# kowaalczyk/reformer-tts

Measured on AMD Instinct MI355X. Metric: mel-frames/sec training step, LJSpeech-shape batch, higher is better.
Workload: dtype bf16; 1 GPU; config/baseline.yml full Reformer-TTS training step (enc 3 / dec 3 layers, d=512, LSH 8 rounds, buckets 64/128), per-GPU batch 12, text 200->256, mel 1024x80; global_batch=12, parallelism=dp1, reversible_recompute=full

## Files before the change

reformer-tts_amd/csrc/gemm_tn.hip:

```cpp
#include "rtts_common.h"
#include <stdlib.h>

#define GT_BM 64
#ifndef GT_PAD
#define GT_PAD 64
#endif

typedef __attribute__((ext_vector_type(8))) short gt_short8;

__device__ __forceinline__ bf16x8 gt_tr_frag(const unsigned char* p0, const unsigned char* p1) {
    const short4v lo = __builtin_amdgcn_ds_read_tr16_b64_v4i16((RTTS_LDS short4v*)p0);
    const short4v hi = __builtin_amdgcn_ds_read_tr16_b64_v4i16((RTTS_LDS short4v*)p1);
    const gt_short8 both = {lo[0], lo[1], lo[2], lo[3], hi[0], hi[1], hi[2], hi[3]};
    return __builtin_bit_cast(bf16x8, both);
}

struct GtProb {
    const bf16_t* a;
    const bf16_t* b;
    float* out;
    float* c;
    int64_t lda, ldb, ldo, ldc;
    size_t slab_stride;
    int M, N, K, split, accumulate;
    int wg_start;
    int rb_start;
};
struct GtGroup {
    GtProb p[RTTS_GEMM_TN_MAX_GROUP];
    int n;
};

template <int WN, int WK, int TN, int TK>
__global__ __launch_bounds__(64 * WN * WK) void gemm_tn_kernel(const GtGroup grp) {
    constexpr int BN = 32 * TN * WN, BK = 32 * TK * WK, NTHR = 64 * WN * WK;
    constexpr int ROWA = BN * 2 + GT_PAD, ROWB = BK * 2 + GT_PAD;
    constexpr int PA = BN / 8, PB = BK / 8;
    constexpr int ITA = GT_BM * PA / NTHR, ITB = GT_BM * PB / NTHR;
    static_assert(GT_BM * PA % NTHR == 0 && GT_BM * PB % NTHR == 0, "staging must tile");
    extern __shared__ __attribute__((aligned(16))) unsigned char smem[];
    unsigned char* As = smem;
    unsigned char* Bs = smem + 2 * GT_BM * ROWA;

    int pi = 0;
#pragma unroll
    for (int i = 1; i < RTTS_GEMM_TN_MAX_GROUP; ++i)
        if (i < grp.n && (int)blockIdx.x >= grp.p[i].wg_start) pi = i;
    const GtProb& P = grp.p[pi];
    const bf16_t* __restrict__ a = P.a;
    const bf16_t* __restrict__ b = P.b;
    float* __restrict__ out = P.out;
    const int64_t lda = P.lda, ldb = P.ldb, ldo = P.ldo;
    const int M = P.M, K = P.K, split = P.split, accumulate = P.accumulate;
    const size_t slab_stride = P.slab_stride;
    const int blk = (int)blockIdx.x - P.wg_start;

    const int tiles_k = K / BK;
    const int tile = blk / split, sp = blk % split;
    const int n0 = (tile / tiles_k) * BN, k0 = (tile % tiles_k) * BK;
    const int st_all = M / GT_BM, st_base = st_all / split, st_rem = st_all % split;
    const int nstage = st_base + (sp < st_rem ? 1 : 0);
    const int m_begin = (sp * st_base + min(sp, st_rem)) * GT_BM;

    const int tid = threadIdx.x, lane = tid & 63, wave = tid >> 6;
    const int wn = wave / WK, wk = wave % WK;
    const int hh = lane >> 5;
    const int trq = (lane & 15) >> 2, trp = lane & 3, trc = (lane >> 4) & 1;

    const int arow = tid / PA, apiece = tid % PA, brow = tid / PB, bpiece = tid % PB;
    static_assert(ITA <= 4 && ITB <= 4, "staging registers");
    uint4 ra0, ra1, ra2, ra3, rb0, rb1, rb2, rb3;
#define GT_LD(reg, base, ld, step, it, IT) \
    if constexpr ((it) < (IT)) reg = *reinterpret_cast<const uint4*>((base) + (size_t)((it) * (step)) * (ld))
#define GT_ST(reg, base, bstep, it, IT) \
    if constexpr ((it) < (IT)) *reinterpret_cast<uint4*>((base) + (it) * (bstep)) = reg
#define GT_LOAD_STAGE(stage)                                                              \
    do {                                                                                  \
        const size_t m_ = (size_t)m_begin + (size_t)(stage) * GT_BM;                      \
        const bf16_t* pa_ = a + (m_ + arow) * lda + n0 + apiece * 8;                      \
        const bf16_t* pb_ = b + (m_ + brow) * ldb + k0 + bpiece * 8;                      \
        GT_LD(ra0, pa_, lda, NTHR / PA, 0, ITA); GT_LD(ra1, pa_, lda, NTHR / PA, 1, ITA); \
        GT_LD(ra2, pa_, lda, NTHR / PA, 2, ITA); GT_LD(ra3, pa_, lda, NTHR / PA, 3, ITA); \
        GT_LD(rb0, pb_, ldb, NTHR / PB, 0, ITB); GT_LD(rb1, pb_, ldb, NTHR / PB, 1, ITB); \
        GT_LD(rb2, pb_, ldb, NTHR / PB, 2, ITB); GT_LD(rb3, pb_, ldb, NTHR / PB, 3, ITB); \
    } while (0)
#define GT_STORE_STAGE(buf)                                                               \
    do {                                                                                  \
        unsigned char* pa_ = As + ((buf) * GT_BM + arow) * ROWA + apiece * 16;            \
        unsigned char* pb_ = Bs + ((buf) * GT_BM + brow) * ROWB + bpiece * 16;            \
        GT_ST(ra0, pa_, (NTHR / PA) * ROWA, 0, ITA); GT_ST(ra1, pa_, (NTHR / PA) * ROWA, 1, ITA); \
        GT_ST(ra2, pa_, (NTHR / PA) * ROWA, 2, ITA); GT_ST(ra3, pa_, (NTHR / PA) * ROWA, 3, ITA); \
        GT_ST(rb0, pb_, (NTHR / PB) * ROWB, 0, ITB); GT_ST(rb1, pb_, (NTHR / PB) * ROWB, 1, ITB); \
        GT_ST(rb2, pb_, (NTHR / PB) * ROWB, 2, ITB); GT_ST(rb3, pb_, (NTHR / PB) * ROWB, 3, ITB); \
    } while (0)

    f32x16 acc[TN][TK];
#pragma unroll
    for (int i = 0; i < TN; ++i)
#pragma unroll
        for (int j = 0; j < TK; ++j) acc[i][j] = (f32x16){0};

    GT_LOAD_STAGE(0);
    GT_STORE_STAGE(0);
    __syncthreads();
    for (int s = 0; s < nstage; ++s) {
        const int buf = s & 1;
        if (s + 1 < nstage) GT_LOAD_STAGE(s + 1);
        const unsigned char* Ab = As + buf * GT_BM * ROWA;
        const unsigned char* Bb = Bs + buf * GT_BM * ROWB;
#define GT_FRAGS(AF, BF, ks_)                                                                   \
    do {                                                                                        \
        const int mr_ = (ks_) * 16 + 8 * hh + trq;                                              \
        _Pragma("unroll") for (int t = 0; t < TN; ++t) {                                        \
            const int ca_ = (wn * 32 * TN + t * 32 + 16 * trc + 4 * trp) * 2;                   \
            AF[t] = gt_tr_frag(Ab + mr_ * ROWA + ca_, Ab + (mr_ + 4) * ROWA + ca_);             \
        }                                                                                       \
        _Pragma("unroll") for (int t = 0; t < TK; ++t) {                                        \
            const int cb_ = (wk * 32 * TK + t * 32 + 16 * trc + 4 * trp) * 2;                   \
            BF[t] = gt_tr_frag(Bb + mr_ * ROWB + cb_, Bb + (mr_ + 4) * ROWB + cb_);             \
        }                                                                                       \
    } while (0)
#define GT_MFMAS(AF, BF)                                                                        \
    _Pragma("unroll") for (int i = 0; i < TN; ++i)                                              \
        _Pragma("unroll") for (int j = 0; j < TK; ++j)                                          \
            acc[i][j] = __builtin_amdgcn_mfma_f32_32x32x16_bf16(AF[i], BF[j], acc[i][j], 0, 0, 0)
        bf16x8 af0[TN], bf0[TK], af1[TN], bf1[TK];
        GT_FRAGS(af0, bf0, 0);
        GT_FRAGS(af1, bf1, 1);
        __builtin_amdgcn_sched_barrier(0);
        GT_MFMAS(af0, bf0);
        __builtin_amdgcn_sched_barrier(0);
        GT_FRAGS(af0, bf0, 2);
        __builtin_amdgcn_sched_barrier(0);
        GT_MFMAS(af1, bf1);
        __builtin_amdgcn_sched_barrier(0);
        GT_FRAGS(af1, bf1, 3);
        __builtin_amdgcn_sched_barrier(0);
        GT_MFMAS(af0, bf0);
        __builtin_amdgcn_sched_barrier(0);
        GT_MFMAS(af1, bf1);
        static_assert(GT_BM == 64, "four k-steps per stage");
        if (s + 1 < nstage) GT_STORE_STAGE(buf ^ 1);
        __syncthreads();
    }
#undef GT_LOAD_STAGE
#undef GT_STORE_STAGE
#undef GT_LD
#undef GT_ST
#undef GT_FRAGS
#undef GT_MFMAS

    float* dst = out + (split > 1 ? (size_t)sp * slab_stride : 0);
    const bool add = (split == 1) && accumulate;
#pragma unroll
    for (int i = 0; i < TN; ++i)
#pragma unroll
        for (int j = 0; j < TK; ++j) {
            const int nb = n0 + wn * 32 * TN + i * 32 + 4 * hh;
            const int kc = k0 + wk * 32 * TK + j * 32 + (lane & 31);
#pragma unroll
            for (int e = 0; e < 16; ++e) {
                float* p = dst + (size_t)(nb + (e & 3) + 8 * (e >> 2)) * ldo + kc;
                *p = add ? *p + acc[i][j][e] : acc[i][j][e];
            }
        }
}

#define GT_RS 32
#ifndef GT_NST
#define GT_NST 4
#endif

template <int WN, int WK, int TN, int TK>
__global__ __launch_bounds__(64 * WN * WK) void gemm_tn_ring_kernel(const GtGroup grp) {
    constexpr int BN = 32 * TN * WN, BK = 32 * TK * WK, NTHR = 64 * WN * WK, NWAVE = WN * WK;
    static_assert(BN == 256 && BK == 256 && NWAVE == 8, "ring variant: 256 x 256 tile, 8 waves");
    constexpr int ROWB = 512;
    constexpr int STAGE = GT_RS * ROWB;
    extern __shared__ __attribute__((aligned(16))) unsigned char smem[];
    unsigned char* As = smem;
    unsigned char* Bs = smem + GT_NST * STAGE;

    int pi = 0;
#pragma unroll
    for (int i = 1; i < RTTS_GEMM_TN_MAX_GROUP; ++i)
        if (i < grp.n && (int)blockIdx.x >= grp.p[i].wg_start) pi = i;
    const GtProb& P = grp.p[pi];
    const bf16_t* __restrict__ a = P.a;
    const bf16_t* __restrict__ b = P.b;
    float* __restrict__ out = P.out;
    const int64_t lda = P.lda, ldb = P.ldb, ldo = P.ldo;
    const int M = P.M, K = P.K, split = P.split, accumulate = P.accumulate;
    const size_t slab_stride = P.slab_stride;
    const int blk = (int)blockIdx.x - P.wg_start;
    const int tiles_k = K / BK;
    const int tile = blk / split, sp = blk % split;
    const int n0 = (tile / tiles_k) * BN, k0 = (tile % tiles_k) * BK;
    const int st_all = M / GT_RS, st_base = st_all / split, st_rem = st_all % split;
    const int nstage = st_base + (sp < st_rem ? 1 : 0);
    const int m_begin = (sp * st_base + min(sp, st_rem)) * GT_RS;

    const int tid = threadIdx.x, lane = tid & 63, wave = __builtin_amdgcn_readfirstlane(tid >> 6);
    const int wn = wave / WK, wk = wave % WK;
    const int hh = lane >> 5;
    const int trq = (lane & 15) >> 2, trp = lane & 3, trc = (lane >> 4) & 1;

    const bf16_t* srcA[2];
    const bf16_t* srcB[2];
#pragma unroll
    for (int i = 0; i < 2; ++i) {
        const int row = 4 * wave + 2 * i + (lane >> 5);
        const int pp = lane & 31;
        const int col = ((((pp >> 2) ^ (row & 3)) << 6) + ((pp & 3) << 4)) >> 1;
        srcA[i] = a + ((size_t)m_begin + row) * lda + n0 + col;
        srcB[i] = b + ((size_t)m_begin + row) * ldb + k0 + col;
    }
#define GT_ISSUE(stage_)                                                                                              \
    do {                                                                                                              \
        const int buf_ = (stage_) % GT_NST;                                                                           \
        const size_t mo_ = (size_t)(stage_) * GT_RS;                                                                  \
        _Pragma("unroll") for (int i = 0; i < 2; ++i) {                                                               \
            __builtin_amdgcn_global_load_lds((const __attribute__((address_space(1))) void*)(srcA[i] + mo_ * lda),    \
                                             (RTTS_LDS void*)(As + buf_ * STAGE + (4 * wave + 2 * i) * ROWB), 16, 0, 0); \
            __builtin_amdgcn_global_load_lds((const __attribute__((address_space(1))) void*)(srcB[i] + mo_ * ldb),    \
                                             (RTTS_LDS void*)(Bs + buf_ * STAGE + (4 * wave + 2 * i) * ROWB), 16, 0, 0); \
        }                                                                                                             \
    } while (0)

    f32x16 acc[TN][TK];
#pragma unroll
    for (int i = 0; i < TN; ++i)
#pragma unroll
        for (int j = 0; j < TK; ++j) acc[i][j] = (f32x16){0};

    int offA[TN], offB[TK];
#pragma unroll
    for (int t = 0; t < TN; ++t) {
        const int cb = (wn * 32 * TN + t * 32 + 16 * trc + 4 * trp) * 2;
        offA[t] = (8 * hh + trq) * ROWB + ((((cb >> 6) ^ trq) << 6) | (cb & 63));
    }
#pragma unroll
    for (int t = 0; t < TK; ++t) {
        const int cb = (wk * 32 * TK + t * 32 + 16 * trc + 4 * trp) * 2;
        offB[t] = (8 * hh + trq) * ROWB + ((((cb >> 6) ^ trq) << 6) | (cb & 63));
    }

    constexpr int AHEAD = GT_NST - 1;
    static_assert(AHEAD >= 2 && AHEAD <= 4, "ring depth 3..5");
#pragma unroll
    for (int i = 0; i < AHEAD; ++i)
        if (i < nstage) GT_ISSUE(i);
    for (int s = 0; s < nstage; ++s) {
        const int later = min(AHEAD - 1, nstage - 1 - s);
        if (later >= 3) __builtin_amdgcn_s_waitcnt(0x0F7C);
        else if (later == 2) __builtin_amdgcn_s_waitcnt(0x0F78);
        else if (later == 1) __builtin_amdgcn_s_waitcnt(0x0F74);
        else __builtin_amdgcn_s_waitcnt(0x0F70);
        asm volatile("s_barrier" ::: "memory");
        if (s + AHEAD < nstage) GT_ISSUE(s + AHEAD);
        const unsigned char* Ab = As + (s % GT_NST) * STAGE;
        const unsigned char* Bb = Bs + (s % GT_NST) * STAGE;
        const uint32_t abase = (uint32_t)(uintptr_t)(RTTS_LDS unsigned char*)Ab;
        const uint32_t bbase = (uint32_t)(uintptr_t)(RTTS_LDS unsigned char*)Bb;
        short4v al[2][TN], ah[2][TN], bl[2][TK], bh[2][TK];
#define GT_TR(dst, addr, off) asm volatile("ds_read_b64_tr_b16 %0, %1 offset:%2" : "=v"(dst) : "v"(addr), "n"(off))
#pragma unroll
        for (int t = 0; t < TN; ++t) {
            const uint32_t ad = abase + offA[t];
            GT_TR(al[0][t], ad, 0);
            GT_TR(ah[0][t], ad, 4 * ROWB);
            GT_TR(al[1][t], ad, 16 * ROWB);
            GT_TR(ah[1][t], ad, 20 * ROWB);
        }
#pragma unroll
        for (int t = 0; t < TK; ++t) {
            const uint32_t ad = bbase + offB[t];
            GT_TR(bl[0][t], ad, 0);
            GT_TR(bh[0][t], ad, 4 * ROWB);
            GT_TR(bl[1][t], ad, 16 * ROWB);
            GT_TR(bh[1][t], ad, 20 * ROWB);
        }
#undef GT_TR
        static_assert(TN == 2 && TK == 4, "operand list of the wait below");
        asm volatile("s_waitcnt lgkmcnt(0)"
                     : "+v"(al[0][0]), "+v"(ah[0][0]), "+v"(al[1][0]), "+v"(ah[1][0]), "+v"(al[0][1]), "+v"(ah[0][1]), "+v"(al[1][1]),
                       "+v"(ah[1][1]), "+v"(bl[0][0]), "+v"(bh[0][0]), "+v"(bl[1][0]), "+v"(bh[1][0]), "+v"(bl[0][1]), "+v"(bh[0][1]),
                       "+v"(bl[1][1]), "+v"(bh[1][1]), "+v"(bl[0][2]), "+v"(bh[0][2]), "+v"(bl[1][2]), "+v"(bh[1][2]), "+v"(bl[0][3]),
                       "+v"(bh[0][3]), "+v"(bl[1][3]), "+v"(bh[1][3]));
        bf16x8 af0[TN], bf0[TK], af1[TN], bf1[TK];
#pragma unroll
        for (int t = 0; t < TN; ++t) {
            const gt_short8 f0 = {al[0][t][0], al[0][t][1], al[0][t][2], al[0][t][3], ah[0][t][0], ah[0][t][1], ah[0][t][2], ah[0][t][3]};
            const gt_short8 f1 = {al[1][t][0], al[1][t][1], al[1][t][2], al[1][t][3], ah[1][t][0], ah[1][t][1], ah[1][t][2], ah[1][t][3]};
            af0[t] = __builtin_bit_cast(bf16x8, f0);
            af1[t] = __builtin_bit_cast(bf16x8, f1);
        }
#pragma unroll
        for (int t = 0; t < TK; ++t) {
            const gt_short8 f0 = {bl[0][t][0], bl[0][t][1], bl[0][t][2], bl[0][t][3], bh[0][t][0], bh[0][t][1], bh[0][t][2], bh[0][t][3]};
            const gt_short8 f1 = {bl[1][t][0], bl[1][t][1], bl[1][t][2], bl[1][t][3], bh[1][t][0], bh[1][t][1], bh[1][t][2], bh[1][t][3]};
            bf0[t] = __builtin_bit_cast(bf16x8, f0);
            bf1[t] = __builtin_bit_cast(bf16x8, f1);
        }
#pragma unroll
        for (int i = 0; i < TN; ++i)
#pragma unroll
            for (int j = 0; j < TK; ++j) acc[i][j] = __builtin_amdgcn_mfma_f32_32x32x16_bf16(af0[i], bf0[j], acc[i][j], 0, 0, 0);
#pragma unroll
        for (int i = 0; i < TN; ++i)
#pragma unroll
            for (int j = 0; j < TK; ++j) acc[i][j] = __builtin_amdgcn_mfma_f32_32x32x16_bf16(af1[i], bf1[j], acc[i][j], 0, 0, 0);
    }
#undef GT_ISSUE

    float* dst = out + (split > 1 ? (size_t)sp * slab_stride : 0);
    const bool add = (split == 1) && accumulate;
#pragma unroll
    for (int i = 0; i < TN; ++i)
#pragma unroll
        for (int j = 0; j < TK; ++j) {
            const int nb = n0 + wn * 32 * TN + i * 32 + 4 * hh;
            const int kc = k0 + wk * 32 * TK + j * 32 + (lane & 31);
#pragma unroll
            for (int e = 0; e < 16; ++e) {
                float* p = dst + (size_t)(nb + (e & 3) + 8 * (e >> 2)) * ldo + kc;
                *p = add ? *p + acc[i][j][e] : acc[i][j][e];
            }
        }
}

__global__ __launch_bounds__(256) void slab_reduce_kernel(const GtGroup grp) {
    int pi = 0;
#pragma unroll
    for (int i = 1; i < RTTS_GEMM_TN_MAX_GROUP; ++i)
        if (i < grp.n && (int)blockIdx.x >= grp.p[i].rb_start) pi = i;
    const GtProb& P = grp.p[pi];
    if (P.split == 1) return;
    const size_t i4 = (size_t)((int)blockIdx.x - P.rb_start) * blockDim.x + threadIdx.x;
    const size_t total4 = P.slab_stride / 4;
    if (i4 >= total4) return;
    const size_t e = i4 * 4;
    const int n = (int)(e / P.K), k = (int)(e % P.K);
    const float* __restrict__ slabs = P.out;
    float4 s = *reinterpret_cast<const float4*>(slabs + e);
    for (int t = 1; t < P.split; ++t) {
        const float4 v = *reinterpret_cast<const float4*>(slabs + (size_t)t * P.slab_stride + e);
        s.x += v.x; s.y += v.y; s.z += v.z; s.w += v.w;
    }
    float4* dst = reinterpret_cast<float4*>(P.c + (size_t)n * P.ldc + k);
    if (P.accumulate) {
        const float4 o = *dst;
        s.x += o.x; s.y += o.y; s.z += o.z; s.w += o.w;
    }
    *dst = s;
}

template <int WN, int WK, int TN, int TK>
static int gt_launch(const GtGroup& grp, int wg, hipStream_t s) {
    constexpr int BN = 32 * TN * WN, BK = 32 * TK * WK;
    const size_t lds = 2 * GT_BM * (BN * 2 + GT_PAD) + 2 * GT_BM * (BK * 2 + GT_PAD);
    static RttsLdsState st = {};
    RTTS_ENSURE_LDS("rtts_gemm_tn", (gemm_tn_kernel<WN, WK, TN, TK>), lds, st);
    hipLaunchKernelGGL((gemm_tn_kernel<WN, WK, TN, TK>), dim3(wg), dim3(64 * WN * WK), lds, s, grp);
    return 0;
}

static bool gt_c_overlap(const rtts_gemm_tn_problem& p, const rtts_gemm_tn_problem& q) {
    const uintptr_t bp = (uintptr_t)p.c, bq = (uintptr_t)q.c;
    const uintptr_t ep = bp + ((uintptr_t)(p.N - 1) * (uintptr_t)p.ldc + (uintptr_t)p.K) * sizeof(float);
    const uintptr_t eq = bq + ((uintptr_t)(q.N - 1) * (uintptr_t)q.ldc + (uintptr_t)q.K) * sizeof(float);
    if (bq >= ep || bp >= eq) return false;
    if (p.ldc != q.ldc) return true;
    const rtts_gemm_tn_problem& lo = bp <= bq ? p : q;
    const rtts_gemm_tn_problem& hi = bp <= bq ? q : p;
    const int64_t d = (int64_t)(((uintptr_t)hi.c - (uintptr_t)lo.c) / sizeof(float));
    const int64_t r = d / lo.ldc, s = d % lo.ldc;
    if (s < lo.K) return true;
    return s + hi.K > lo.ldc && r + 1 < lo.N;
}

extern "C" int rtts_gemm_tn_grouped(const rtts_gemm_tn_problem* problems, int n, float* slab_ws, int64_t slab_ws_floats, void* stream) {
    RTTS_ENTER(stream);
    RTTS_REQUIRE(problems && n > 0 && n <= RTTS_GEMM_TN_MAX_GROUP, "rtts_gemm_tn_grouped: 1..%d problems", RTTS_GEMM_TN_MAX_GROUP);
    GtGroup grp;
    grp.n = n;
    bool big = getenv("RTTS_GEMM_TN_SMALL_TILES") == nullptr;
    long long flops = 0;
    for (int i = 0; i < n; ++i) {
        const rtts_gemm_tn_problem& q = problems[i];
        RTTS_REQUIRE(q.a && q.b && q.c, "rtts_gemm_tn: null pointer");
        RTTS_REQUIRE(q.N > 0 && q.K > 0 && q.M > 0 && q.N % 128 == 0 && q.K % 128 == 0 && q.M % GT_BM == 0,
                     "rtts_gemm_tn: need N %% 128 == 0, K %% 128 == 0, M %% 64 == 0 (got M=%d N=%d K=%d)", q.M, q.N, q.K);
        RTTS_REQUIRE(q.lda >= q.N && q.ldb >= q.K && q.ldc >= q.K && q.lda % 8 == 0 && q.ldb % 8 == 0 && q.ldc % 4 == 0,
                     "rtts_gemm_tn: bad leading dimensions");
        RTTS_REQUIRE((((uintptr_t)q.a | (uintptr_t)q.b | (uintptr_t)q.c) & 15) == 0, "rtts_gemm_tn: buffers must be 16-byte aligned");
        big = big && q.N % 256 == 0 && q.K % 256 == 0;
        flops += 2LL * q.M * q.N * q.K;
    }
    for (int i = 1; i < n; ++i)
        for (int j = 0; j < i; ++j)
            RTTS_REQUIRE(!gt_c_overlap(problems[j], problems[i]),
                         "rtts_gemm_tn_grouped: problems %d and %d write overlapping parts of C (launch them one after the other)", j, i);
    static const long long big_min = [] { const char* e = getenv("RTTS_GEMM_TN_BIG_MIN_GFLOP"); return (e ? atoll(e) : 40LL) * 1000000000LL; }();
    if (flops < big_min) big = false;
    const int bt = big ? 256 : 128;
    int total_tiles = 0;
    for (int i = 0; i < n; ++i) total_tiles += (problems[i].N / bt) * (problems[i].K / bt);
    const int wg_target = big ? 320 : 640;
    int want = 1;
    while (total_tiles * want * 2 <= wg_target) want *= 2;
    int wg = 0, rb = 0;
    size_t slab_used = 0;
    bool any_split = false;
    for (int i = 0; i < n; ++i) {
        const rtts_gemm_tn_problem& q = problems[i];
        GtProb& P = grp.p[i];
        const int tiles = (q.N / bt) * (q.K / bt), stages = q.M / GT_BM;
        const size_t slab = (size_t)q.N * q.K;
        int split = 1;
        while (split < want && split * 2 <= stages / 4) split *= 2;
        while (split > 1 && (!slab_ws || slab_used + slab * split > (size_t)slab_ws_floats)) split /= 2;
        P.a = (const bf16_t*)q.a; P.b = (const bf16_t*)q.b; P.c = q.c;
        P.lda = q.lda; P.ldb = q.ldb; P.ldc = q.ldc;
        P.M = q.M; P.N = q.N; P.K = q.K; P.split = split; P.accumulate = q.accumulate;
        P.slab_stride = slab;
        P.wg_start = wg;
        P.rb_start = rb;
        wg += tiles * split;
        if (split > 1) {
            P.out = slab_ws + slab_used;
            P.ldo = q.K;
            slab_used += slab * split;
            rb += (int)((slab / 4 + 255) / 256);
            any_split = true;
        } else {
            P.out = q.c;
            P.ldo = q.ldc;
        }
    }
    hipStream_t s = (hipStream_t)stream;
    static const bool ring = getenv("RTTS_GEMM_TN_NO_RING") == nullptr;
    if (big && ring) {
        const size_t lds = 2 * GT_NST * GT_RS * 512;
        static RttsLdsState st = {};
        RTTS_ENSURE_LDS("rtts_gemm_tn", (gemm_tn_ring_kernel<4, 2, 2, 4>), lds, st);
        hipLaunchKernelGGL((gemm_tn_ring_kernel<4, 2, 2, 4>), dim3(wg), dim3(512), lds, s, grp);
    } else if (big) {
        if (gt_launch<4, 2, 2, 4>(grp, wg, s)) return -1;
    } else if (gt_launch<2, 2, 2, 2>(grp, wg, s)) return -1;
    if (any_split) hipLaunchKernelGGL(slab_reduce_kernel, dim3(rb), dim3(256), 0, s, grp);
    RTTS_LAUNCH_CHECK("rtts_gemm_tn");
    return 0;
}

extern "C" int rtts_gemm_tn(const void* a, int64_t lda, const void* b, int64_t ldb, int M, int N, int K, float* c, int64_t ldc,
                            int accumulate, float* slab_ws, int64_t slab_ws_floats, void* stream) {
    RTTS_ENTER(stream);
    rtts_gemm_tn_problem q;
    q.a = a; q.lda = lda; q.b = b; q.ldb = ldb; q.c = c; q.ldc = ldc;
    q.M = M; q.N = N; q.K = K; q.accumulate = accumulate;
    return rtts_gemm_tn_grouped(&q, 1, slab_ws, slab_ws_floats, stream);
}
```

reformer-tts_amd/engine.py:

```python
from __future__ import annotations

from typing import List, Optional

import os

import torch

from . import _lib, ops
from ._seeds import next_seed, seed_base
from .model.lsh_attention import LSHSelfAttention


STASH_ATTENTION = True
STASH_BLOCK_OUTPUT = True
STASH_PROJECTIONS = True
STASH_STREAMS = True
_NO_G = object()


def _streams_kept() -> bool:
    return STASH_STREAMS and STASH_ATTENTION and STASH_BLOCK_OUTPUT and STASH_PROJECTIONS


RECOMPUTE_MODES = ("full", "attention-stash", "output-stash", "projection-stash", "stash")
# ... 355 lines not shown
def gemm_dgrad_delta(dy: torch.Tensor, w: torch.Tensor, out: torch.Tensor, t: int, heads: int):
    m = dy.shape[0]
    n = w.shape[1]
    if n != heads * 64 or m % t:
        raise ValueError("gemm_dgrad_delta: N must be 64 x heads and M a multiple of T")
    dout = torch.empty(m, n, dtype=torch.bfloat16, device=dy.device)
    delta = torch.empty((m // t) * heads, t, dtype=torch.float32, device=dy.device)
    arr = (_lib.GemmNtProblem * 1)()
    flop = _nt_problem(arr[0], dy, w, True, dout, None, 5, aux=out, aux_out=delta, t=t, h=heads)
    ev = ops.TIMING.start(f"rtts_gemm_nt/{m}x{n}x{dy.shape[1]}")
    _lib.call("rtts_gemm_nt_grouped", arr, 1, 1, _s())
    ops.TIMING.stop(ev, flop)
    return dout, delta


def dgrad_delta_ok(m: int, n: int) -> bool:
    return (m % 192 == 0 and n % 128 == 0) or (m % 128 == 0 and n % 64 == 0)


FUSE_DELTA = os.environ.get("RTTS_FUSE_DELTA", "1") != "0"
GROUP_XATTN = os.environ.get("RTTS_GROUP_XATTN", "1") != "0"
GROUP_XATTN_BWD = os.environ.get("RTTS_GROUP_XATTN_BWD", "0") == "1"

_SLAB_FLOATS = 16 * 1024 * 1024

DEFER_WGRAD = True
WGRAD_FLUSH_PER_LAYER = os.environ.get("RTTS_WGRAD_FLUSH", "layer") == "layer"
WGRAD_MAX_PENDING = 64
STAMPS = None


def stamp(name: str) -> None:
    if STAMPS is None:
        return
    buf, names = STAMPS
    slot = names.setdefault(name, len(names))
    _lib.call("rtts_debug_stamp", buf.data_ptr(), slot, _s())


JOIN_STREAMS = os.environ.get("RTTS_JOIN_STREAMS", "1") != "0"
COPY_STREAMS = os.environ.get("RTTS_STREAM_COPIES", "0") == "1"


STEAL = None


def run_handed_over(steal) -> int:
    main = torch.cuda.current_stream()
    n = 0
    for ev, entries in steal["pending"]:
        main.wait_event(ev)
        for gv, dy, x in entries:
            dy.record_stream(main)
            x.record_stream(main)
        n += _launch_wgrads(entries, _s())
    del steal["pending"][:]
    return n


def _c_overlap(g1: torch.Tensor, g2: torch.Tensor) -> bool:
    b1, b2 = g1.data_ptr(), g2.data_ptr()
    e1 = b1 + ((g1.shape[0] - 1) * g1.stride(0) + g1.shape[1]) * 4
    e2 = b2 + ((g2.shape[0] - 1) * g2.stride(0) + g2.shape[1]) * 4
    if b2 >= e1 or b1 >= e2:
        return False
    if g1.stride(0) != g2.stride(0):
        return True
    lo, hi = (g1, g2) if b1 <= b2 else (g2, g1)
    r, s = divmod((hi.data_ptr() - lo.data_ptr()) // 4, lo.stride(0))
    return s < lo.shape[1] or (s + hi.shape[1] > lo.stride(0) and r + 1 < lo.shape[0])


def _launch_wgrads(entries, stream: int) -> int:
    groups = launch_groups(entries, _lib.GEMM_TN_MAX_GROUP, lambda a, b: _c_overlap(a[0], b[0]))
    for group in groups:
        arr = (_lib.GemmTnProblem * len(group))()
        for e, (gv, dy, x) in zip(arr, group):
            e.a, e.lda, e.b, e.ldb, e.c, e.ldc = dy.data_ptr(), dy.stride(0), x.data_ptr(), x.stride(0), gv.data_ptr(), gv.stride(0)
            e.M, e.N, e.K, e.accumulate = dy.shape[0], dy.shape[1], x.shape[1], 1
        ws = _slab_ws(group[0][1].device, stream)
        _lib.call("rtts_gemm_tn_grouped", arr, len(group), ws.data_ptr(), ws.numel(), stream)
    return len(groups)


def _final_flush():
    flush_wgrad()


def _slab_ws(device, stream: Optional[int] = None):
    stream = torch.cuda.current_stream(device).cuda_stream if stream is None else stream
    key = ("slab", torch.device(device), stream)
    if key not in _WS._cache:
        _WS._cache[key] = torch.empty(_SLAB_FLOATS, dtype=torch.float32, device=device)
    return _WS._cache[key]


def _queue_final_flush():
    q = _queue()
    if not q.flush_queued:
        try:
            torch.autograd.Variable._execution_engine.queue_callback(_final_flush)
            q.flush_queued = True
        except RuntimeError:
            pass


def flush_wgrad(colsums: bool = True, keys=None):
    for q in _all_queues(keys):
        q.flush_queued = False
        if not len(q):
            continue
        with torch.cuda.device(q.device):
            if colsums or len(q.colsums) >= _lib.COLSUM_MAX_GROUP - 8:
                flush_colsum(q)
            elif q.colsums and (q.device, q.stream) == (torch.cuda.current_device(), _s()):
                _queue_final_flush()
            pending = q.wgrads
            steal = STEAL
            if steal is not None and steal.get("armed") and pending and (q.device, q.stream) == steal["src"]:
                ev = torch.cuda.Event()
                ev.record(steal["src_stream"])
                steal["pending"].append((ev, list(pending)))
                del pending[:]
            if pending:
                entries = list(pending)
                del pending[:]
                _launch_wgrads(entries, q.stream)
            for hook in FLUSH_HOOKS:
                hook(q)


def discard_pending(keys=None) -> int:
    n = 0
    for q in _all_queues(keys):
        n += len(q)
        q.clear()
    return n


FLUSH_HOOKS = []


def pending_wgrads() -> int:
    return len(_queue().wgrads)


def pending_all(keys=None) -> int:
    return sum(len(q) for q in _all_queues(keys))


def wgrad(grad_view: torch.Tensor, dy: torch.Tensor, x: torch.Tensor, accumulate: bool = True):
    m, n = dy.shape
    k = x.shape[1]
    if n % 128 == 0 and k % 128 == 0 and m % 64 == 0 and dy.stride(1) == 1 and x.stride(1) == 1 and grad_view.stride(1) == 1:
        if DEFER_WGRAD and accumulate:
            _queue().wgrads.append((grad_view, dy, x))
            _queue_final_flush()
            return
        ws = _slab_ws(dy.device)
        _lib.call("rtts_gemm_tn", dy.data_ptr(), dy.stride(0), x.data_ptr(), x.stride(0), m, n, k, grad_view.data_ptr(),
                  grad_view.stride(0), int(accumulate), ws.data_ptr(), ws.numel(), _s())
    elif n % 128 == 0 and m % 64 == 0 and m >= 4096 and k < 128 and dy.stride(1) == 1:
        xp = torch.zeros(m, 128, dtype=x.dtype, device=x.device)
        xp[:, :k].copy_(x)
        tmp = torch.empty(n, 128, dtype=torch.float32, device=x.device)
        ws = _slab_ws(dy.device)
        _lib.call("rtts_gemm_tn", dy.data_ptr(), dy.stride(0), xp.data_ptr(), 128, m, n, 128, tmp.data_ptr(), 128, 0, ws.data_ptr(),
                  ws.numel(), _s())
        if accumulate:
            grad_view.add_(tmp[:, :k])
        else:
            grad_view.copy_(tmp[:, :k])
    else:
        _lib.note_general_path("weight gradient", f"dW {n} x {k} over {m} rows does not tile (N, K % 128, M % 64): library GEMM")
        if accumulate:
            grad_view.add_(torch.mm(dy.t(), x, out_dtype=torch.float32))
        else:
            grad_view.copy_(torch.mm(dy.t(), x, out_dtype=torch.float32))


def _keep_streams(keep, slot, acc, inp, xn, mean, rstd, fresh=False):
    if not keep:
        if fresh:
            out = slot["acc_out"] = torch.empty_like(acc)
            return out
        return None
    out = torch.empty_like(acc)
    slot.update(inp=inp, pre=(xn, mean, rstd), acc_out=out)
    if STASH_BLOCK_OUTPUT:
        slot["g"] = None
    return out


class LSHExec:

    def __init__(self, withnorm):
        self.norm = withnorm.norm
        self.layer: LSHSelfAttention = withnorm.fn.layer
        self._own_slot = {}

    @staticmethod
    def supported(withnorm) -> bool:
        return withnorm.fn.layer.dim % 64 == 0

    def _wqkv(self):
        lyr = self.layer
        a, b = _bf16(lyr.toqk.weight), _bf16(lyr.tov.weight)
        if _adjacent(a, b):
            return torch.as_strided(a, (2 * a.shape[0], a.shape[1]), (a.shape[1], 1))
        return torch.cat([a, b], dim=0)

    def _wqkv_grad(self):
        lyr = self.layer
        ga, gb = _grad(lyr.toqk.weight), _grad(lyr.tov.weight)
        if _adjacent(ga, gb):
            return torch.as_strided(ga, (2 * ga.shape[0], ga.shape[1]), (ga.shape[1], 1)), None
        return None, (ga, gb)

    def _internals(self, inp, b, t, mask, st, stash=None, g=None, pre=None, qkv=None, adrop=None):
        lyr = self.layer
        e = lyr.dim
        if t <= lyr.full_attn_thres:
            raise NotImplementedError("full-attention shortcut (T <= full_attn_thres) is outside the HIP path")
        xn, mean, rstd = pre if pre is not None else ln_fwd(inp, self.norm)
        wqkv = self._wqkv()
        if qkv is None:
            qkv = gemm(xn, wqkv).view(b, t, 2 * e)
        if st is None:
            rot = lyr._rotations(qkv, t // lyr.bucket_size)
            st, _, _ = ops.lsh_hash_sort(qkv[..., :e], rot, lyr.heads, lyr.bucket_size)
        lyr.last_st = st
        if stash is not None:
            out, lse_tot = stash
        else:
            o, lse = ops.lsh_attn_fwd(qkv[..., :e], qkv[..., e:], st, lyr.heads, lyr.bucket_size, lyr.causal, mask, adrop)
            out, lse_tot = ops.lsh_combine_fwd(o, lse, b, lyr.heads)
        if g is None:
            g = gemm(out.view(b * t, e), _bf16(lyr.to_out.weight))
        return xn, mean, rstd, wqkv, qkv, st, out, lse_tot, g

    def forward(self, acc, inp, b, t, mask=None, pre=None, next_norm=None, slot=None, keep_streams=False, fresh_acc=False, **_):
        slot = self._own_slot if slot is None else slot
        pa = getattr(self.layer, "dropout", 0.0) if self.layer.training else 0.0
        adrop = (pa, next_seed()) if pa > 0.0 else None
        xn, mean, rstd, _, qkv, st, out, lse_tot, g = self._internals(inp, b, t, mask, None, pre=pre, adrop=adrop)
        p = self.layer.post_attn_dropout.p if self.layer.training else 0.0
        slot.clear()
        slot.update(st=st, stash=(out, lse_tot) if STASH_ATTENTION else None, g=g if STASH_BLOCK_OUTPUT else None,
                    qkv=qkv if STASH_PROJECTIONS else None, drop=(p, next_seed()) if p > 0.0 else None, adrop=adrop)
        return residual(acc, g, self.layer.to_out.bias, 1.0, next_norm, slot["drop"], out=_keep_streams(keep_streams, slot, acc, inp, xn, mean, rstd, fresh_acc))

    def backward(self, acc, inp, d_acc, d_inp, b, t, mask=None, pre=None, next_norm=None, pre_cast=None, next_cast=None, slot=None,
                 d_src=None, join=None, **_):
        slot = self._own_slot if slot is None else slot
        if "st" not in slot:
            raise RuntimeError("LSHExec.backward: no forward state for this call (backward run twice, or without its forward)")
        lyr = self.layer
        e = lyr.dim
        kept = "inp" in slot
        if kept:
            inp, pre = slot["inp"], slot["pre"]
        adrop = slot.get("adrop")
        xn, mean, rstd, wqkv, qkv, st, out, lse_tot, g = self._internals(inp, b, t, mask, slot["st"], slot["stash"],
                                                                         _NO_G if kept else slot["g"], pre, slot["qkv"], adrop)
        drop = slot["drop"]
        slot.clear()
        post = None if kept else residual(acc, g, lyr.to_out.bias, -1.0, next_norm, drop)
        dyb = _out_grad(d_acc, _grad(lyr.to_out.bias), drop, pre_cast)
        out2 = out.view(b * t, e)
        wgrad(_grad(lyr.to_out.weight), dyb, out2)
        delta = None
        if FUSE_DELTA and e == 64 * lyr.heads and dgrad_delta_ok(b * t, e):
            dout, delta = gemm_dgrad_delta(dyb, _bf16(lyr.to_out.weight), out2, t, lyr.heads)
            dout = dout.view(b, t, e)
        else:
            dout = gemm(dyb, _bf16(lyr.to_out.weight), kn=True).view(b, t, e)
        dqkv = torch.empty_like(qkv)
        ops.lsh_attn_bwd(qkv[..., :e], qkv[..., e:], st, out, dout, lse_tot, lyr.heads, lyr.bucket_size, lyr.causal, mask,
                         dqkv=(dqkv[..., :e], dqkv[..., e:]), drop=adrop, delta=delta)
        dqkv2 = dqkv.view(b * t, 2 * e)
        gview, pair = self._wqkv_grad()
        if gview is not None:
            wgrad(gview, dqkv2, xn)
        else:
            _lib.note_general_path("weight gradient", "toqk / tov gradients are not neighbours in one buffer: library GEMM")
            full = torch.mm(dqkv2.t(), xn, out_dtype=torch.float32)
            pair[0].add_(full[:e])
            pair[1].add_(full[e:])
        dxn = gemm(dqkv2, wqkv, kn=True)
        return post, ln_bwd(dxn, inp, mean, rstd, self.norm, d_inp, next_cast, dx_in=d_src, join=join)


class FFNExec:

    def __init__(self, mod):
        wn = mod.fn if hasattr(mod, "chunks") else mod
        self.norm = wn.norm
        self.l1, self.l2 = wn.fn.net[0], wn.fn.net[3]
        self._own_slot = {}

    @staticmethod
    def supported(mod) -> bool:
        wn = mod.fn if hasattr(mod, "chunks") else mod
        lin1, lin2 = wn.fn.net[0], wn.fn.net[3]
        return wn.fn.net[2].p == 0.0 and all(v % 64 == 0 for v in (lin1.in_features, lin1.out_features, lin2.out_features))

    def _internals(self, inp, g=None, pre=None, h=None):
        xn, mean, rstd = pre if pre is not None else ln_fwd(inp, self.norm)
        if h is None:
            words = gate_words(xn.shape[0], self.l1.weight.shape[0], xn.device)
            h = (gemm(xn, _bf16(self.l1.weight), bias=self.l1.bias, relu=True, words=words), words)
        if g is None:
            g = gemm(h[0], _bf16(self.l2.weight))
        return xn, mean, rstd, h, g

    def forward(self, acc, inp, b, t, pre=None, next_norm=None, slot=None, keep_streams=False, fresh_acc=False, **_):
        slot = self._own_slot if slot is None else slot
        xn, mean, rstd, h, g = self._internals(inp, pre=pre)
        slot.clear()
        slot.update(g=g if STASH_BLOCK_OUTPUT else None, h=h if STASH_PROJECTIONS else None)
        return residual(acc, g, self.l2.bias, 1.0, next_norm, out=_keep_streams(keep_streams, slot, acc, inp, xn, mean, rstd, fresh_acc))

    def backward(self, acc, inp, d_acc, d_inp, b, t, pre=None, next_norm=None, pre_cast=None, next_cast=None, slot=None, d_src=None,
                 join=None, **_):
        slot = self._own_slot if slot is None else slot
        if "g" not in slot:
            raise RuntimeError("FFNExec.backward: no forward state for this call (backward run twice, or without its forward)")
# ... 388 lines not shown
```

Before: 1.947 million mel-frames/s.

## Vectorize gemm_tn epilogue stores and support ragged K without padding copies

The weight-gradient GEMM epilogue now swaps the MFMA operands so each lane holds contiguous output columns. Pairs of lanes exchange halves via DPP so every lane writes 16-byte vectors, replacing 16 scattered scalar stores per tile. The kernel also masks B loads and stores past K, so K only needs to be a multiple of 8. This removes the host-side zero-padding, temporary buffer and add/copy path for narrow weight gradients such as the 80-wide mel projection. The cost is extra predication and cross-lane shuffles, and narrow K is excluded from the deferred batched wgrad queue.

```diff
diff --git a/reformer-tts_amd/csrc/gemm_tn.hip b/reformer-tts_amd/csrc/gemm_tn.hip
--- a/reformer-tts_amd/csrc/gemm_tn.hip
+++ b/reformer-tts_amd/csrc/gemm_tn.hip
@@ -6,7 +6,75 @@
 #define GT_PAD 64
 #endif
 
+#ifndef GT_EPI
+#define GT_EPI 2
+#endif
+#ifndef GT_WT
+#define GT_WT RTTS_WT_STORES
+#endif
+
 typedef __attribute__((ext_vector_type(8))) short gt_short8;
+
+#if GT_EPI
+#define GT_MFMA(af, bf, c) __builtin_amdgcn_mfma_f32_32x32x16_bf16(bf, af, c, 0, 0, 0)
+#else
+#define GT_MFMA(af, bf, c) __builtin_amdgcn_mfma_f32_32x32x16_bf16(af, bf, c, 0, 0, 0)
+#endif
+
+__device__ __forceinline__ void gt_store4(float* p, f32x4 v, const bool add) {
+    if (add) v += *reinterpret_cast<const f32x4*>(p);
+#if GT_WT
+    rtts_store16_out(p, __builtin_bit_cast(uint4, v));
+#else
+    *reinterpret_cast<f32x4*>(p) = v;
+#endif
+}
+
+__device__ __forceinline__ f32x4 gt_lane_xor1(const f32x4 v) {
+    f32x4 r;
+#pragma unroll
+    for (int c = 0; c < 4; ++c) r[c] = __int_as_float(__builtin_amdgcn_update_dpp(0, __float_as_int(v[c]), 0xB1, 0xF, 0xF, true));
+    return r;
+}
+
+__device__ __forceinline__ void gt_store_tile(float* __restrict__ dst, const int64_t ldo, const int n_tile, const int k_tile, const int K,
+                                              const f32x16& acc, const bool add, const int lane) {
+    const int hh = lane >> 5;
+#if GT_EPI == 0
+    const int kc = k_tile + (lane & 31);
+    if (kc >= K) return;
+#pragma unroll
+    for (int e = 0; e < 16; ++e) {
+        float* p = dst + (size_t)(n_tile + 4 * hh + (e & 3) + 8 * (e >> 2)) * ldo + kc;
+        *p = add ? *p + acc[e] : acc[e];
+    }
+#else
+    const int n = n_tile + (lane & 31);
+    const f32x4 x0 = {acc[0], acc[1], acc[2], acc[3]}, x1 = {acc[4], acc[5], acc[6], acc[7]};
+    const f32x4 x2 = {acc[8], acc[9], acc[10], acc[11]}, x3 = {acc[12], acc[13], acc[14], acc[15]};
+#if GT_EPI == 1
+    float* row = dst + (size_t)n * ldo + k_tile + 4 * hh;
+    if (k_tile + 4 * hh < K) gt_store4(row, x0, add);
+    if (k_tile + 4 * hh + 8 < K) gt_store4(row + 8, x1, add);
+    if (k_tile + 4 * hh + 16 < K) gt_store4(row + 16, x2, add);
+    if (k_tile + 4 * hh + 24 < K) gt_store4(row + 24, x3, add);
+#else
+    const bool odd = (lane & 1) != 0;
+    const f32x4 r0 = gt_lane_xor1(odd ? x0 : x1), r1 = gt_lane_xor1(odd ? x2 : x3);
+    const int kk = k_tile + 4 * hh + (odd ? 8 : 0);
+    float* even_row = dst + (size_t)(n & ~1) * ldo + kk;
+    float* odd_row = dst + (size_t)(n | 1) * ldo + kk;
+    if (kk < K) {
+        gt_store4(even_row, odd ? r0 : x0, add);
+        gt_store4(odd_row, odd ? x1 : r0, add);
+    }
+    if (kk + 16 < K) {
+        gt_store4(even_row + 16, odd ? r1 : x2, add);
+        gt_store4(odd_row + 16, odd ? x3 : r1, add);
+    }
+#endif
+#endif
+}
 
 __device__ __forceinline__ bf16x8 gt_tr_frag(const unsigned char* p0, const unsigned char* p1) {
     const short4v lo = __builtin_amdgcn_ds_read_tr16_b64_v4i16((RTTS_LDS short4v*)p0);
@@ -55,7 +123,7 @@
     const size_t slab_stride = P.slab_stride;
     const int blk = (int)blockIdx.x - P.wg_start;
 
-    const int tiles_k = K / BK;
+    const int tiles_k = (K + BK - 1) / BK;
     const int tile = blk / split, sp = blk % split;
     const int n0 = (tile / tiles_k) * BN, k0 = (tile % tiles_k) * BK;
     const int st_all = M / GT_BM, st_base = st_all / split, st_rem = st_all % split;
@@ -69,9 +137,12 @@
 
     const int arow = tid / PA, apiece = tid % PA, brow = tid / PB, bpiece = tid % PB;
     static_assert(ITA <= 4 && ITB <= 4, "staging registers");
-    uint4 ra0, ra1, ra2, ra3, rb0, rb1, rb2, rb3;
-#define GT_LD(reg, base, ld, step, it, IT) \
-    if constexpr ((it) < (IT)) reg = *reinterpret_cast<const uint4*>((base) + (size_t)((it) * (step)) * (ld))
+    uint4 ra0, ra1, ra2, ra3;
+    const uint4 zero4 = {0u, 0u, 0u, 0u};
+    uint4 rb0 = zero4, rb1 = zero4, rb2 = zero4, rb3 = zero4;
+    const bool b_in = k0 + bpiece * 8 < K;
+#define GT_LD(reg, base, ld, step, it, IT, ok) \
+    if constexpr ((it) < (IT)) if (ok) reg = *reinterpret_cast<const uint4*>((base) + (size_t)((it) * (step)) * (ld))
 #define GT_ST(reg, base, bstep, it, IT) \
     if constexpr ((it) < (IT)) *reinterpret_cast<uint4*>((base) + (it) * (bstep)) = reg
 #define GT_LOAD_STAGE(stage)                                                              \
@@ -79,10 +150,10 @@
         const size_t m_ = (size_t)m_begin + (size_t)(stage) * GT_BM;                      \
         const bf16_t* pa_ = a + (m_ + arow) * lda + n0 + apiece * 8;                      \
         const bf16_t* pb_ = b + (m_ + brow) * ldb + k0 + bpiece * 8;                      \
-        GT_LD(ra0, pa_, lda, NTHR / PA, 0, ITA); GT_LD(ra1, pa_, lda, NTHR / PA, 1, ITA); \
-        GT_LD(ra2, pa_, lda, NTHR / PA, 2, ITA); GT_LD(ra3, pa_, lda, NTHR / PA, 3, ITA); \
-        GT_LD(rb0, pb_, ldb, NTHR / PB, 0, ITB); GT_LD(rb1, pb_, ldb, NTHR / PB, 1, ITB); \
-        GT_LD(rb2, pb_, ldb, NTHR / PB, 2, ITB); GT_LD(rb3, pb_, ldb, NTHR / PB, 3, ITB); \
+        GT_LD(ra0, pa_, lda, NTHR / PA, 0, ITA, true); GT_LD(ra1, pa_, lda, NTHR / PA, 1, ITA, true); \
+        GT_LD(ra2, pa_, lda, NTHR / PA, 2, ITA, true); GT_LD(ra3, pa_, lda, NTHR / PA, 3, ITA, true); \
+        GT_LD(rb0, pb_, ldb, NTHR / PB, 0, ITB, b_in); GT_LD(rb1, pb_, ldb, NTHR / PB, 1, ITB, b_in); \
+        GT_LD(rb2, pb_, ldb, NTHR / PB, 2, ITB, b_in); GT_LD(rb3, pb_, ldb, NTHR / PB, 3, ITB, b_in); \
     } while (0)
 #define GT_STORE_STAGE(buf)                                                               \
     do {                                                                                  \
@@ -123,7 +194,7 @@
 #define GT_MFMAS(AF, BF)                                                                        \
     _Pragma("unroll") for (int i = 0; i < TN; ++i)                                              \
         _Pragma("unroll") for (int j = 0; j < TK; ++j)                                          \
-            acc[i][j] = __builtin_amdgcn_mfma_f32_32x32x16_bf16(AF[i], BF[j], acc[i][j], 0, 0, 0)
+            acc[i][j] = GT_MFMA(AF[i], BF[j], acc[i][j])
         bf16x8 af0[TN], bf0[TK], af1[TN], bf1[TK];
         GT_FRAGS(af0, bf0, 0);
         GT_FRAGS(af1, bf1, 1);
@@ -155,15 +226,8 @@
 #pragma unroll
     for (int i = 0; i < TN; ++i)
 #pragma unroll
-        for (int j = 0; j < TK; ++j) {
-            const int nb = n0 + wn * 32 * TN + i * 32 + 4 * hh;
-            const int kc = k0 + wk * 32 * TK + j * 32 + (lane & 31);
-#pragma unroll
-            for (int e = 0; e < 16; ++e) {
-                float* p = dst + (size_t)(nb + (e & 3) + 8 * (e >> 2)) * ldo + kc;
-                *p = add ? *p + acc[i][j][e] : acc[i][j][e];
-            }
-        }
+        for (int j = 0; j < TK; ++j)
+            gt_store_tile(dst, ldo, n0 + wn * 32 * TN + i * 32, k0 + wk * 32 * TK + j * 32, K, acc[i][j], add, lane);
 }
 
 #define GT_RS 32
@@ -305,11 +369,11 @@
 #pragma unroll
         for (int i = 0; i < TN; ++i)
 #pragma unroll
-            for (int j = 0; j < TK; ++j) acc[i][j] = __builtin_amdgcn_mfma_f32_32x32x16_bf16(af0[i], bf0[j], acc[i][j], 0, 0, 0);
+            for (int j = 0; j < TK; ++j) acc[i][j] = GT_MFMA(af0[i], bf0[j], acc[i][j]);
 #pragma unroll
         for (int i = 0; i < TN; ++i)
 #pragma unroll
-            for (int j = 0; j < TK; ++j) acc[i][j] = __builtin_amdgcn_mfma_f32_32x32x16_bf16(af1[i], bf1[j], acc[i][j], 0, 0, 0);
+            for (int j = 0; j < TK; ++j) acc[i][j] = GT_MFMA(af1[i], bf1[j], acc[i][j]);
     }
 #undef GT_ISSUE
 
@@ -318,15 +382,8 @@
 #pragma unroll
     for (int i = 0; i < TN; ++i)
 #pragma unroll
-        for (int j = 0; j < TK; ++j) {
-            const int nb = n0 + wn * 32 * TN + i * 32 + 4 * hh;
-            const int kc = k0 + wk * 32 * TK + j * 32 + (lane & 31);
-#pragma unroll
-            for (int e = 0; e < 16; ++e) {
-                float* p = dst + (size_t)(nb + (e & 3) + 8 * (e >> 2)) * ldo + kc;
-                *p = add ? *p + acc[i][j][e] : acc[i][j][e];
-            }
-        }
+        for (int j = 0; j < TK; ++j)
+            gt_store_tile(dst, ldo, n0 + wn * 32 * TN + i * 32, k0 + wk * 32 * TK + j * 32, K, acc[i][j], add, lane);
 }
 
 __global__ __launch_bounds__(256) void slab_reduce_kernel(const GtGroup grp) {
@@ -389,8 +446,8 @@
     for (int i = 0; i < n; ++i) {
         const rtts_gemm_tn_problem& q = problems[i];
         RTTS_REQUIRE(q.a && q.b && q.c, "rtts_gemm_tn: null pointer");
-        RTTS_REQUIRE(q.N > 0 && q.K > 0 && q.M > 0 && q.N % 128 == 0 && q.K % 128 == 0 && q.M % GT_BM == 0,
-                     "rtts_gemm_tn: need N %% 128 == 0, K %% 128 == 0, M %% 64 == 0 (got M=%d N=%d K=%d)", q.M, q.N, q.K);
+        RTTS_REQUIRE(q.N > 0 && q.K > 0 && q.M > 0 && q.N % 128 == 0 && q.K % 8 == 0 && q.M % GT_BM == 0,
+                     "rtts_gemm_tn: need N %% 128 == 0, K %% 8 == 0, M %% 64 == 0 (got M=%d N=%d K=%d)", q.M, q.N, q.K);
         RTTS_REQUIRE(q.lda >= q.N && q.ldb >= q.K && q.ldc >= q.K && q.lda % 8 == 0 && q.ldb % 8 == 0 && q.ldc % 4 == 0,
                      "rtts_gemm_tn: bad leading dimensions");
         RTTS_REQUIRE((((uintptr_t)q.a | (uintptr_t)q.b | (uintptr_t)q.c) & 15) == 0, "rtts_gemm_tn: buffers must be 16-byte aligned");
@@ -405,7 +462,7 @@
     if (flops < big_min) big = false;
     const int bt = big ? 256 : 128;
     int total_tiles = 0;
-    for (int i = 0; i < n; ++i) total_tiles += (problems[i].N / bt) * (problems[i].K / bt);
+    for (int i = 0; i < n; ++i) total_tiles += (problems[i].N / bt) * ((problems[i].K + bt - 1) / bt);
     const int wg_target = big ? 320 : 640;
     int want = 1;
     while (total_tiles * want * 2 <= wg_target) want *= 2;
@@ -415,7 +472,7 @@
     for (int i = 0; i < n; ++i) {
         const rtts_gemm_tn_problem& q = problems[i];
         GtProb& P = grp.p[i];
-        const int tiles = (q.N / bt) * (q.K / bt), stages = q.M / GT_BM;
+        const int tiles = (q.N / bt) * ((q.K + bt - 1) / bt), stages = q.M / GT_BM;
         const size_t slab = (size_t)q.N * q.K;
         int split = 1;
         while (split < want && split * 2 <= stages / 4) split *= 2;
diff --git a/reformer-tts_amd/engine.py b/reformer-tts_amd/engine.py
--- a/reformer-tts_amd/engine.py
+++ b/reformer-tts_amd/engine.py
@@ -531,27 +531,19 @@
 def wgrad(grad_view: torch.Tensor, dy: torch.Tensor, x: torch.Tensor, accumulate: bool = True):
     m, n = dy.shape
     k = x.shape[1]
-    if n % 128 == 0 and k % 128 == 0 and m % 64 == 0 and dy.stride(1) == 1 and x.stride(1) == 1 and grad_view.stride(1) == 1:
-        if DEFER_WGRAD and accumulate:
+    tiles = n % 128 == 0 and m % 64 == 0 and dy.stride(1) == 1 and x.stride(1) == 1 and grad_view.stride(1) == 1
+    narrow = (k % 128 != 0 and k % 8 == 0 and dy.stride(0) % 8 == 0 and x.stride(0) % 8 == 0 and grad_view.stride(0) % 4 == 0
+              and (dy.data_ptr() | x.data_ptr() | grad_view.data_ptr()) % 16 == 0)
+    if tiles and (k % 128 == 0 or narrow):
+        if DEFER_WGRAD and accumulate and k % 128 == 0:
             _queue().wgrads.append((grad_view, dy, x))
             _queue_final_flush()
             return
         ws = _slab_ws(dy.device)
         _lib.call("rtts_gemm_tn", dy.data_ptr(), dy.stride(0), x.data_ptr(), x.stride(0), m, n, k, grad_view.data_ptr(),
                   grad_view.stride(0), int(accumulate), ws.data_ptr(), ws.numel(), _s())
-    elif n % 128 == 0 and m % 64 == 0 and m >= 4096 and k < 128 and dy.stride(1) == 1:
-        xp = torch.zeros(m, 128, dtype=x.dtype, device=x.device)
-        xp[:, :k].copy_(x)
-        tmp = torch.empty(n, 128, dtype=torch.float32, device=x.device)
-        ws = _slab_ws(dy.device)
-        _lib.call("rtts_gemm_tn", dy.data_ptr(), dy.stride(0), xp.data_ptr(), 128, m, n, 128, tmp.data_ptr(), 128, 0, ws.data_ptr(),
-                  ws.numel(), _s())
-        if accumulate:
-            grad_view.add_(tmp[:, :k])
-        else:
-            grad_view.copy_(tmp[:, :k])
     else:
-        _lib.note_general_path("weight gradient", f"dW {n} x {k} over {m} rows does not tile (N, K % 128, M % 64): library GEMM")
+        _lib.note_general_path("weight gradient", f"dW {n} x {k} over {m} rows does not tile (N % 128, K % 8, M % 64): library GEMM")
         if accumulate:
             grad_view.add_(torch.mm(dy.t(), x, out_dtype=torch.float32))
         else:
```

Result: no change. 1.935 million mel-frames/s (-0.6%).
